# cnkuangshi/LightCTR

Hardware: AMD Instinct MI355X
Metric: examples/sec (whole node), FM training on synthetic Criteo-shaped sparse (higher is better)
Workload: dtype fp32; 1 GPU; model=FM k=16, ftrl fused update, global_batch=65536, num_features=16777216, num_fields=39, parallelism=single-gpu, hipGraph

## Files before the change

lightctr_amd/models/fm.py:

```python

from __future__ import annotations

from dataclasses import dataclass

import torch

from ..ops import fm_ref
from ..ops._extension import require_hip_ops, sort_ids, sort_ids_rec
from ..utils.checks import validate_csr_batch
from ..utils.metrics import auc_score


@dataclass
class FMHyper:
    num_features: int
    k: int = 16
    optimizer: str = "adagrad"
    lr: float = 0.1
    eps: float = 1e-8
    l2: float = 1e-5
    ftrl_alpha: float = 0.15
    ftrl_beta: float = 1.0
    ftrl_l1: float = 1e-4
    ftrl_l2: float = 1e-4
    ftrl_v: str = "adagrad"
    init_sigma: float = 0.01
    seed: int = 1234


class FMModel:

    def __init__(self, hyper: FMHyper, device: str = "cpu",
                 max_batch_nnz: int = 1 << 22):
        self.h = hyper
        self.device = torch.device(device)
        F, K = hyper.num_features, hyper.k
        assert K in (4, 8, 16, 32, 64), "K must divide the 64-lane wavefront"
        g = torch.Generator().manual_seed(hyper.seed)
        self.W = torch.zeros(F, device=self.device)
        self.V = (
            torch.randn(F, K, generator=g) * hyper.init_sigma
        ).to(self.device)
        self.gradW = torch.zeros_like(self.W)
        self.gradV = torch.zeros_like(self.V)
        self.nW = torch.zeros_like(self.W)
        self.nV = torch.zeros_like(self.V)
        if hyper.optimizer == "ftrl":
            self.zW = torch.zeros_like(self.W)
            self.zV = torch.zeros_like(self.V)
        nwords = (F + 63) // 64
        self.touched = torch.zeros(nwords, dtype=torch.int64, device=self.device)
        cap = min(F, max_batch_nnz)
        self.uniq = torch.zeros(cap, dtype=torch.int32, device=self.device)
        self.count = torch.zeros(1, dtype=torch.int32, device=self.device)
        self._use_hip = self.device.type == "cuda"
        self.backward_mode = "segment"
        self.segment_cap = 256
        self.fused_apply = False
        if self._use_hip:
            require_hip_ops()

    def forward(self, row_ptr, fids, vals):
        if self._use_hip:
            ops = require_hip_ops()
            pred, sumVX = ops.fm_forward(row_ptr, fids, vals, self.W, self.V)
        else:
            pred, sumVX = fm_ref.fm_forward_ref(row_ptr, fids, vals, self.W, self.V)
        return pred, sumVX

    def predict_proba(self, row_ptr, fids, vals):
        pred, _ = self.forward(row_ptr, fids, vals)
        return torch.sigmoid(torch.clamp(pred, -16, 16))

    def train_step(self, row_ptr, fids, vals, labels) -> torch.Tensor:
        B = row_ptr.numel() - 1
        scale = 1.0 / B
        validate_csr_batch(row_ptr, fids, vals, self.h.num_features)
        if self._use_hip:
            ops = require_hip_ops()
            if (self.backward_mode in ("segment", "segment_list")
                    and not self.fused_apply):
                tiled = (self.backward_mode == "segment"
                         and self._cap_tiles(ops))
                loss, dpred, sumVX, rec = ops.fm_forward_train(
                    row_ptr, fids, vals, self.W, self.V, labels, scale,
                    reset=self.count if tiled else None)
                self._segment_backward(ops, fids, sumVX, dpred, rec, tiled)
                return loss
            pred, sumVX = ops.fm_forward(row_ptr, fids, vals, self.W, self.V)
            loss, dpred = ops.logloss_grad(pred, labels, scale)
            if (self.backward_mode == "segment_emit"
                    and not self.fused_apply):
                self._segment_emit_backward(ops, row_ptr, fids, vals, sumVX,
                                            dpred)
                return loss
            if self.backward_mode in ("sorted", "segment", "segment_list",
                                      "segment_emit"):
                sorted_fids, perm = sort_ids(fids, self.h.num_features)
                gw, gv = ops.fm_backward_emit(row_ptr, fids, vals, self.V,
                                              sumVX, dpred)
                if self.fused_apply:
                    if (self.h.optimizer == "ftrl"
                            and self.h.ftrl_v == "adagrad"):
                        ops.fm_sorted_apply_fused(
                            sorted_fids, perm, gw, gv, self.gradW,
                            self.gradV, self.touched, self.W, self.V,
                            self.nW, self.nV, self.zW, None, 3,
                            self.h.ftrl_alpha, self.h.ftrl_beta,
                            self.h.ftrl_l1, self.h.ftrl_l2,
                            v_lr=self.h.lr, v_eps=self.h.eps,
                            v_l2=self.h.l2)
                    elif self.h.optimizer == "ftrl":
                        ops.fm_sorted_apply_fused(
                            sorted_fids, perm, gw, gv, self.gradW,
                            self.gradV, self.touched, self.W, self.V,
                            self.nW, self.nV, self.zW, self.zV, 2,
                            self.h.ftrl_alpha, self.h.ftrl_beta,
                            self.h.ftrl_l1, self.h.ftrl_l2)
                    else:
                        ops.fm_sorted_apply_fused(
                            sorted_fids, perm, gw, gv, self.gradW,
                            self.gradV, self.touched, self.W, self.V,
                            self.nW, self.nV, None, None, 1, self.h.lr,
                            self.h.eps, self.h.l2, 0.0)
                else:
                    ops.fm_sorted_apply(sorted_fids, perm, gw, gv,
                                        self.gradW, self.gradV,
                                        self.touched)
            else:
                ops.fm_backward(row_ptr, fids, vals, self.V, sumVX, dpred,
                                self.gradW, self.gradV, self.touched)
            self.count.zero_()
            ops.bitmap_compact(self.touched, self.uniq, self.count)
            live = self.uniq[: min(self.uniq.numel(), fids.numel())]
            self._sparse_apply(ops, live)
            return loss
        pred, sumVX = fm_ref.fm_forward_ref(row_ptr, fids, vals, self.W, self.V)
        loss, dpred = fm_ref.logloss_grad_ref(pred, labels, scale)
        gW, gV = fm_ref.fm_backward_ref(row_ptr, fids, vals, self.V, sumVX, dpred)
        self.gradW += gW
        self.gradV += gV
        uniq = torch.unique(fids.long()).int()
        if self.h.optimizer == "ftrl":
            fm_ref.ftrl_apply_ref(uniq, self.W, self.V, self.zW, self.nW,
                                  self.zV, self.nV, self.gradW, self.gradV,
                                  self.h.ftrl_alpha, self.h.ftrl_beta,
                                  self.h.ftrl_l1, self.h.ftrl_l2,
                                  v_adagrad=self.h.ftrl_v == "adagrad",
                                  v_lr=self.h.lr, v_eps=self.h.eps,
                                  v_l2=self.h.l2)
        else:
            fm_ref.adagrad_apply_ref(uniq, self.W, self.V, self.nW, self.nV,
                                     self.gradW, self.gradV, self.h.lr,
                                     self.h.eps, self.h.l2)
        return loss

    def _opt_mode(self) -> int:
        if self.h.optimizer != "ftrl":
            return 1
        return 3 if self.h.ftrl_v == "adagrad" else 2

    def _sparse_apply(self, ops, live):
        if self.h.optimizer == "ftrl":
            ops.fm_ftrl_apply(live, self.count, self.W, self.V,
                              self.zW, self.nW, self.zV, self.nV,
                              self.gradW, self.gradV, self.h.ftrl_alpha,
                              self.h.ftrl_beta, self.h.ftrl_l1,
                              self.h.ftrl_l2,
                              1 if self.h.ftrl_v == "adagrad" else 0,
                              self.h.lr, self.h.eps, self.h.l2)
        else:
            ops.fm_adagrad_apply(live, self.count, self.W, self.V,
                                 self.nW, self.nV, self.gradW, self.gradV,
                                 self.h.lr, self.h.eps, self.h.l2)

    def _cap_tiles(self, ops) -> bool:
        tile, cap = ops.fm_segment_tile(), int(self.segment_cap)
        return cap <= tile and tile % cap == 0

    def _segment_pieces(self, ops, sorted_fids, worklist=True):
        nnz = sorted_fids.numel()
        cap = int(self.segment_cap)
        if worklist:
            lists = tuple(ops.segment_worklist(sorted_fids, cap, self.count))
        else:
            lists = (cap,)
        spill = self.uniq[: min(self.uniq.numel(), nnz // cap + 1)]
        mode = self._opt_mode()
        if mode == 1:
            knobs = (self.h.lr, self.h.eps, self.h.l2, 0.0)
        else:
            knobs = (self.h.ftrl_alpha, self.h.ftrl_beta, self.h.ftrl_l1,
                     self.h.ftrl_l2)
        tail = (*lists, self.gradW, self.gradV, spill,
                self.count, self.W, self.V, self.nW, self.nV,
                self.zW if mode != 1 else None,
                self.zV if mode == 2 else None, mode, *knobs)
        kw = dict(v_lr=self.h.lr, v_eps=self.h.eps, v_l2=self.h.l2)
        return spill, tail, kw

    def _segment_backward(self, ops, fids, sumVX, dpred, rec, tiled):
        if fids.numel() == 0:
            return
        sorted_fids, sorted_rec = sort_ids_rec(fids, rec,
                                               self.h.num_features)
        spill, tail, kw = self._segment_pieces(ops, sorted_fids,
                                               worklist=not tiled)
        reduce = (ops.fm_segment_tile_rec if tiled
                  else ops.fm_segment_apply_rec)
        reduce(sorted_fids, sorted_rec, sumVX, dpred, *tail, **kw)
        self._sparse_apply(ops, spill)

    def _segment_emit_backward(self, ops, row_ptr, fids, vals, sumVX, dpred):
        if fids.numel() == 0:
            return
        sorted_fids, perm = sort_ids(fids, self.h.num_features)
        gw, gv = ops.fm_backward_emit(row_ptr, fids, vals, self.V, sumVX,
                                      dpred)
        spill, tail, kw = self._segment_pieces(ops, sorted_fids)
        ops.fm_segment_apply(sorted_fids, perm, tail[0], tail[1], gw, gv,
                             *tail[2:], **kw)
        self._sparse_apply(ops, spill)

    def state_dict(self) -> dict:
        d = {"W": self.W, "V": self.V, "nW": self.nW, "nV": self.nV,
             "hyper": self.h.__dict__}
        if self.h.optimizer == "ftrl":
            d["zW"], d["zV"] = self.zW, self.zV
        return d

    def save(self, path: str) -> None:
        torch.save(self.state_dict(), path)

    def load(self, path: str) -> None:
        d = torch.load(path, map_location=self.device, weights_only=True)
        self.W.copy_(d["W"])
        self.V.copy_(d["V"])
        self.nW.copy_(d["nW"])
        self.nV.copy_(d["nV"])
        if self.h.optimizer == "ftrl" and "zW" in d:
            self.zW.copy_(d["zW"])
            self.zV.copy_(d["zV"])


class FMTrainer:

    def __init__(self, dataset, hyper: FMHyper, device: str = "cpu",
                 batch_size: int = 256, epochs: int = 5):
        self.ds = dataset
        self.model = FMModel(hyper, device=device)
        self.batch_size = batch_size
        self.epochs = epochs
        self.device = torch.device(device)

    def train(self, log=print):
        ds = self.ds.to(self.device)
        N = ds.num_rows
        for ep in range(self.epochs):
            total_loss = 0.0
            nb = 0
            for s in range(0, N, self.batch_size):
                e = min(s + self.batch_size, N)
                b = ds.slice_rows(s, e)
                loss = self.model.train_step(b.row_ptr, b.fids, b.vals, b.labels)
                total_loss += float(loss.mean())
                nb += 1
            if log:
                log(f"epoch {ep}: loss={total_loss / max(nb, 1):.5f}")
        return self

    def evaluate(self, dataset=None) -> dict:
        ds = (dataset or self.ds).to(self.device)
        p = self.model.predict_proba(ds.row_ptr, ds.fids, ds.vals)
        loss = torch.nn.functional.binary_cross_entropy(
            p.clamp(1e-7, 1 - 1e-7), ds.labels
        )
        return {
            "auc": auc_score(p.cpu(), ds.labels.cpu()),
            "logloss": float(loss),
            "accuracy": float(((p > 0.5) == (ds.labels > 0.5)).float().mean()),
        }
```

lightctr_amd/ops/_extension.py:

```python

from __future__ import annotations

import torch

_hip_ops = None
_import_error: Exception | None = None

try:
    from . import _hip_ops as _ext

    _hip_ops = _ext
except ImportError as e:
    _import_error = e


def has_hip_ops() -> bool:
    return _hip_ops is not None


def require_hip_ops():
    if _hip_ops is None:
        raise ImportError(
            "lightctr_amd HIP extension (_hip_ops) is not built but a GPU "
            "op was requested. Build it in-tree with "
            "`PYTORCH_ROCM_ARCH=gfx950 python setup.py build_ext --inplace`. "
            f"Original import error: {_import_error!r}"
        )
    return _hip_ops


class _LazyOps:

    def __getattr__(self, name):
        return getattr(require_hip_ops(), name)


hip_ops = _LazyOps()


def sort_ids(fids, upper: int):
    end_bit = max(1, int(upper - 1).bit_length())
    return require_hip_ops().radix_sort_index(fids, end_bit)


def sort_ids_rec(fids, rec, upper: int):
    end_bit = max(1, int(upper - 1).bit_length())
    return require_hip_ops().radix_sort_rec(fids, rec, end_bit)
```

lightctr_amd/ops/csrc/bindings.cpp:

```cpp
#include <torch/extension.h>
#include <ATen/cuda/CUDAContext.h>
#include <c10/cuda/CUDAException.h>

#include <cstdint>
#include <cstdio>
#include <cstdlib>
#include <cstring>
#include <limits>
#include <stdexcept>
#include <string>
#include <vector>

#include "launchers.h"

namespace {

#define CHK(x, ...) TORCH_CHECK(x, __VA_ARGS__)

void check_cuda_f32(const at::Tensor& t, const char* name) {
  CHK(t.is_cuda(), name, " must be on GPU");
  CHK(t.scalar_type() == at::kFloat, name, " must be fp32");
  CHK(t.is_contiguous(), name, " must be contiguous");
}

// ... 1030 lines not shown
at::Tensor gemm_bf16(at::Tensor A, at::Tensor Bst,
                     c10::optional<at::Tensor> bias, int64_t M, int64_t N,
                     int64_t K, int64_t transA, int64_t transB, int64_t act,
                     bool emit_bf16) {
  const float* bias_ptr =
      check_gemm_args(A, Bst, bias, M, N, K, transA, transB, act);
  auto C = at::empty({M, N}, A.options().dtype(at::kFloat));
  at::Tensor Cbf;
  void* cbf_ptr = nullptr;
  if (emit_bf16) {
    Cbf = at::empty({M, N}, A.options());
    cbf_ptr = Cbf.data_ptr();
  }
  lightctr::gemm_bf16_launch(A.data_ptr(), Bst.data_ptr(), bias_ptr,
                             C.data_ptr<float>(), cbf_ptr, (int)M, (int)N,
                             (int)K, (int)transA, (int)transB, (int)act,
                             cur_stream());
  return C;
}

std::vector<at::Tensor> gemm_bf16_full(at::Tensor A, at::Tensor Bst,
                                       c10::optional<at::Tensor> bias,
                                       int64_t M, int64_t N, int64_t K,
                                       int64_t transA, int64_t transB,
                                       int64_t act) {
  const float* bias_ptr =
      check_gemm_args(A, Bst, bias, M, N, K, transA, transB, act);
  auto C = at::empty({M, N}, A.options().dtype(at::kFloat));
  auto Cbf = at::empty({M, N}, A.options());
  lightctr::gemm_bf16_launch(A.data_ptr(), Bst.data_ptr(), bias_ptr,
                             C.data_ptr<float>(), Cbf.data_ptr(), (int)M,
                             (int)N, (int)K, (int)transA, (int)transB,
                             (int)act, cur_stream());
  return {C, Cbf};
}

std::vector<at::Tensor> act_backward(at::Tensor dY, at::Tensor Y,
                                     int64_t act) {
  check_cuda_f32(dY, "dY");
  auto dZ = at::empty_like(dY);
  auto dZbf = at::empty_like(dY, dY.options().dtype(at::kBFloat16));
  lightctr::act_backward_launch(dY.data_ptr<float>(), Y.data_ptr<float>(),
                                dZ.data_ptr<float>(), dZbf.data_ptr(),
                                dY.numel(), (int)act, cur_stream());
  return {dZ, dZbf};
}

std::vector<at::Tensor> radix_sort_index(at::Tensor keys, int64_t end_bit) {
  check_cuda_i32(keys, "keys");
  CHK(end_bit >= 1 && end_bit <= 32, "end_bit in [1,32]");
  const int n = (int)keys.numel();
  auto sorted = at::empty_like(keys);
  auto perm = at::empty({n}, keys.options());
  auto iota = at::empty({n}, keys.options());
  lightctr::iota_i32_launch(iota.data_ptr<int>(), n, cur_stream());
  const unsigned long bytes =
      lightctr::radix_sort_pairs_i32_temp_bytes(n, (int)end_bit);
  auto temp = at::empty({(long)bytes}, keys.options().dtype(at::kByte));
  lightctr::radix_sort_pairs_i32_launch(
      temp.data_ptr(), bytes, keys.data_ptr<int>(), sorted.data_ptr<int>(),
      iota.data_ptr<int>(), perm.data_ptr<int>(), n, (int)end_bit,
      cur_stream());
  return {sorted, perm};
}

std::vector<at::Tensor> radix_sort_rec(at::Tensor keys, at::Tensor rec,
                                       int64_t end_bit) {
  check_cuda_i32(keys, "keys");
  CHK(end_bit >= 1 && end_bit <= 32, "end_bit in [1,32]");
  const int n = (int)keys.numel();
  check_cuda_rec(rec, n, "rec");
  auto sorted = at::empty_like(keys);
  auto sorted_rec = at::empty_like(rec);
  if (n == 0) return {sorted, sorted_rec};
  const unsigned long bytes =
      lightctr::radix_sort_pairs_rec_temp_bytes(n, (int)end_bit);
  auto temp = at::empty({(long)bytes}, keys.options().dtype(at::kByte));
  lightctr::radix_sort_pairs_rec_launch(
      temp.data_ptr(), bytes, keys.data_ptr<int>(), sorted.data_ptr<int>(),
      rec.data_ptr<int>(), sorted_rec.data_ptr<int>(), n, (int)end_bit,
      cur_stream());
  return {sorted, sorted_rec};
}

at::Tensor colsum(at::Tensor dZ) {
  check_cuda_f32(dZ, "dZ");
  const int M = (int)dZ.size(0), N = (int)dZ.size(1);
  auto db = at::empty({N}, dZ.options());
  lightctr::colsum_launch(dZ.data_ptr<float>(), db.data_ptr<float>(), M, N,
                          cur_stream());
  return db;
}

at::Tensor to_bf16(at::Tensor x) {
  check_cuda_f32(x, "x");
  auto y = at::empty_like(x, x.options().dtype(at::kBFloat16));
  lightctr::to_bf16_launch(x.data_ptr<float>(), y.data_ptr(), x.numel(),
                           cur_stream());
  return y;
}

void dense_adam(at::Tensor W, at::Tensor grad, at::Tensor m, at::Tensor v,
                c10::optional<at::Tensor> Wbf, c10::optional<at::Tensor> Wtbf,
                double lr, double beta1, double beta2, double eps,
                int64_t step, double l2) {
  check_cuda_f32(W, "W");
  const int rows = (int)W.size(0);
  const int cols = (int)(W.numel() / W.size(0));
  const float bc1 = 1.f - powf((float)beta1, (float)step);
  const float bc2 = 1.f - powf((float)beta2, (float)step);
  lightctr::dense_adam_launch(
      W.data_ptr<float>(), grad.data_ptr<float>(), m.data_ptr<float>(),
      v.data_ptr<float>(), Wbf.has_value() ? Wbf->data_ptr() : nullptr,
      Wtbf.has_value() ? Wtbf->data_ptr() : nullptr, rows, cols, (float)lr,
      (float)beta1, (float)beta2, (float)eps, bc1, bc2, (float)l2,
      cur_stream());
}

void dense_adagrad(at::Tensor W, at::Tensor grad, at::Tensor n,
                   c10::optional<at::Tensor> Wbf,
                   c10::optional<at::Tensor> Wtbf, double lr, double eps,
                   double l2) {
  check_cuda_f32(W, "W");
  const int rows = (int)W.size(0);
  const int cols = (int)(W.numel() / W.size(0));
  lightctr::dense_adagrad_launch(
      W.data_ptr<float>(), grad.data_ptr<float>(), n.data_ptr<float>(),
      Wbf.has_value() ? Wbf->data_ptr() : nullptr,
      Wtbf.has_value() ? Wtbf->data_ptr() : nullptr, rows, cols, (float)lr,
      (float)eps, (float)l2, cur_stream());
}


at::Tensor embed_gather(at::Tensor row_ptr, at::Tensor fids, at::Tensor vals,
                        at::Tensor E, int64_t nf) {
  check_cuda_i32(row_ptr, "row_ptr");
  check_cuda_i32(fids, "fids");
  check_cuda_f32(vals, "vals");
  check_cuda_f32(E, "E");
  CHK(E.dim() == 2, "E must be [F, K]");
  CHK(fids.numel() == vals.numel(), "fids/vals length mismatch");
  CHK(row_ptr.numel() >= 1, "row_ptr must hold B+1 offsets");
  CHK(nf >= 1, "nf must be >= 1");
  const int B = (int)row_ptr.numel() - 1;
  const int K = (int)E.size(1);
  check_embed_k(K);
  auto out = at::empty({B, nf * K}, E.options().dtype(at::kBFloat16));
  lightctr::embed_gather_launch(row_ptr.data_ptr<int>(), fids.data_ptr<int>(),
                                vals.data_ptr<float>(), E.data_ptr<float>(),
                                out.data_ptr(), (int)nf, B, K, cur_stream());
  return out;
}

std::vector<at::Tensor> embed_backward_emit(at::Tensor row_ptr,
                                            at::Tensor vals, at::Tensor dOut,
                                            at::Tensor dwide, int64_t nf,
                                            int64_t K) {
  check_cuda_i32(row_ptr, "row_ptr");
  check_cuda_f32(dOut, "dOut");
  check_cuda_f32(vals, "vals");
  check_cuda_f32(dwide, "dwide");
  check_embed_k(K);
  CHK(nf >= 1, "nf must be >= 1");
  const int B = (int)row_ptr.numel() - 1;
  CHK(dOut.numel() == (int64_t)B * nf * K, "dOut must be [B, nf*K]");
  const auto nnz = vals.numel();
// ... 494 lines not shown
  m.def("fm_segment_tile", &lightctr::fm_segment_tile,
        "entries per block of fm_segment_tile_rec");
  m.def("fm_segment_split", &lightctr::fm_segment_split,
        "longest unit one subgroup sums in fm_segment_tile_rec");
  m.def("ffm_forward", &ffm_forward, "FFM pairwise forward (LDS-staged)");
  m.def("ffm_forward_pp", &ffm_forward_pp, "lane-per-pair FFM forward");
  m.def("ffm_row_emit", &ffm_row_emit,
        "FFM per-row staged fp16 block emit -> (gw, gblocks)",
        py::arg("row_ptr"), py::arg("fields"), py::arg("fids"),
        py::arg("vals"), py::arg("V"), py::arg("dpred"),
        py::arg("scale") = 1.0);
  m.def("ffm_blocks_apply_f16", &ffm_blocks_apply_f16,
        "segment-reduce fp16 blocks into slabs (interior stores), "
        "optionally with the optimizer fused for interior runs",
        py::arg("sorted_fids"), py::arg("perm"), py::arg("gblocks"),
        py::arg("gw"), py::arg("gradW"), py::arg("gradV"),
        py::arg("touched"), py::arg("inv_scale") = 1.0,
        py::arg("opt_mode") = 0, py::arg("V") = py::none(),
        py::arg("W") = py::none(), py::arg("nW") = py::none(),
        py::arg("zW") = py::none(), py::arg("nV") = py::none(),
        py::arg("Vh") = py::none(), py::arg("p0") = 0.0,
        py::arg("p1") = 0.0, py::arg("p2") = 0.0, py::arg("p3") = 0.0,
        py::arg("q0") = 0.0, py::arg("q1") = 0.0, py::arg("q2") = 0.0);
  m.def("ffm_backward", &ffm_backward, "FFM fused pairwise backward scatter");
  m.def("ffm_sorted_backward", &ffm_sorted_backward,
        "FFM sorted segment-reduce backward (LDS block accumulate)");
  m.def("row_index", &row_index, "entry -> row index from row_ptr");
  m.def("ffm_block_lds_bytes", &lightctr::ffm_block_lds_bytes,
        "dynamic LDS per block of ffm_sorted_backward / ffm_block_emit",
        py::arg("nfields"), py::arg("K"));
  m.def("ffm_max_lds_per_block", &lightctr::ffm_max_lds_per_block,
        "per-block LDS limit of the current device, in bytes");
  m.def("ffm_block_emit", &ffm_block_emit,
        "FFM per-entry [nf,K] gradient blocks (wave/entry)");
  m.def("ffm_blocks_apply", &ffm_blocks_apply,
        "segment-reduce sorted FFM blocks into slabs");
  m.def("parse_libffm", &parse_libffm, "native libffm text parser",
        py::arg("path"), py::arg("max_rows") = -1);
  m.def("sparse_adagrad_apply", &sparse_adagrad_apply,
        "generic sparse fused Adagrad (runtime D)",
        py::arg("uniq"), py::arg("count"), py::arg("W"), py::arg("V"),
        py::arg("nW"), py::arg("nV"), py::arg("gradW"), py::arg("gradV"),
        py::arg("lr"), py::arg("eps"), py::arg("l2"),
        py::arg("Vh") = py::none());
  m.def("ps_apply", &ps_apply,
        "PS-side fused updater (sgd/adagrad/dcasgd/dcasgda)");
  m.def("ps_dense_check", &ps_dense_check,
        "PS dense push: non-finite scan of the payload -> flags[0]",
        py::arg("payload"), py::arg("scale"), py::arg("table"),
        py::arg("flags"));
  m.def("ps_dense_apply", &ps_dense_apply,
        "PS dense push: fused decode + updater over the slab, gated on "
        "flags[0]; a gated push bumps flags[1]. flags[0] is only what the "
        "last ps_dense_check left there: call ps_dense_check on the same "
        "payload, on the same stream, immediately before every call (as "
        "DenseTable.apply does) — called alone it acts on a stale flag",
        py::arg("payload"), py::arg("scale"), py::arg("table"),
        py::arg("slab"), py::arg("acc"), py::arg("shadow"),
        py::arg("flags"), py::arg("updater"), py::arg("lr"),
        py::arg("lam"), py::arg("eps"));
  m.def("ps_dense_pack", &ps_dense_pack,
        "PS dense pull: slab -> fp32/fp16 payload (+ shadow = slab)",
        py::arg("slab"), py::arg("shadow"), py::arg("fp16"));
  m.def("sparse_ftrl_apply", &sparse_ftrl_apply,
        "generic sparse fused FTRL (runtime D; optional Adagrad on V)",
        py::arg("uniq"), py::arg("count"), py::arg("W"), py::arg("V"),
        py::arg("zW"), py::arg("nW"), py::arg("zV"), py::arg("nV"),
        py::arg("gradW"), py::arg("gradV"), py::arg("alpha"),
        py::arg("beta"), py::arg("l1"), py::arg("l2"),
        py::arg("v_adagrad") = 0, py::arg("v_lr") = 0.05,
        py::arg("v_eps") = 1e-8, py::arg("v_l2") = 1e-5,
        py::arg("Vh") = py::none());
  m.def("gemm_bf16", &gemm_bf16, "MFMA bf16 GEMM (C fp32), fused bias+act");
  m.def("gemm_bf16_full", &gemm_bf16_full,
        "MFMA bf16 GEMM returning (C fp32, C bf16)");
  m.def("act_backward", &act_backward, "dZ = dY*act'(Y), + bf16 mirror");
  m.def("inv_perm_i32", &inv_perm_i32, "inverse permutation (int32)");
  m.def("radix_sort_index", &radix_sort_index,
        "bit-range radix sort -> (sorted, perm)");
  m.def("radix_sort_rec", &radix_sort_rec,
        "bit-range radix sort with [n,2] int32 records as payload -> "
        "(sorted, sorted_rec)",
        py::arg("keys"), py::arg("rec"), py::arg("end_bit"));
  m.def("colsum", &colsum, "bias gradient column sum");
  m.def("to_bf16", &to_bf16, "f32 -> bf16 convert");
  m.def("dense_adam", &dense_adam, "dense Adam + bf16 mirror refresh");
  m.def("dense_adagrad", &dense_adagrad,
        "dense Adagrad + bf16 mirror refresh");
  m.def("embed_gather", &embed_gather, "concat embedding gather -> bf16");
  m.def("embed_backward_emit", &embed_backward_emit,
        "per-entry embedding grads (gw, gv) for sorted apply");
  m.def("wide_forward", &wide_forward, "LR wide forward sum");
  m.def("w2v_negsample_step", &w2v_negsample_step,
        "fused CBOW negative-sampling train step (Hogwild)");
  m.def("quantile_encode", &quantile_encode, "int8 quantile encode");
  m.def("quantile_decode", &quantile_decode, "int8 quantile decode");
  m.def("lowbit_encode", &lowbit_encode, "1/2-bit sign quantize");
  m.def("lowbit_decode", &lowbit_decode, "1/2-bit dequantize");
  m.def("gbm_hist", &gbm_hist, "GBM per-node (grad,hess) histograms");
  m.def("gbm_forest", &gbm_forest,
        "compiled-forest inference: margin / leaf id / leaf feature id");
  m.def("gbm_forest_chunk_capacity", &lightctr::gbm_forest_chunk_capacity,
        "nodes per LDS chunk of the forest kernel");
  m.def("gbm_forest_max_register_classes",
        &lightctr::gbm_forest_max_register_classes,
        "largest class count with register accumulators");
  m.def("gbm_forest_rows_per_grid", &lightctr::gbm_forest_rows_per_grid,
        "rows one trip of the clamped grid covers");
  m.def("nfm_forward", &nfm_forward,
        "NFM bi-interaction fwd (wide, sumVX, vec, vec_bf16)");
  m.def("nfm_backward_emit", &nfm_backward_emit,
        "NFM per-entry grads for sorted apply");
  m.def("bitmap_compact", &bitmap_compact, "touched bitmap -> fid list");
  m.def("wg_probe", &wg_probe, "wgrad staging/tr-read debug probe");
  m.def("gemm_bf16_variant", &gemm_bf16_variant,
        "launch one named GEMM body directly; returns [C] or [C, Cbf]");
  m.def("gemm_bf16_route", &gemm_bf16_route,
        "name of the GEMM body the default dispatch picks");
  m.def("gemm_wgrad_bf16", &gemm_wgrad_bf16,
        "K-major x K-major wgrad GEMM (tr16 fragment reads)");
  m.def("im2col_bf16", &im2col_bf16,
        "fused unfold -> bf16 GEMM operand [B*L, C*k*k]");
  m.def("col2im", &col2im, "conv data-grad fold (gather form)");
  m.def("auc_hist_add", &auc_hist_add,
        "atomic pos/neg histogram accumulate for AUC");
  m.def("auc_scan", &auc_scan,
        "device scan of the AUC histogram -> {correct, P, N}");
  m.def("fm_adagrad_apply", &fm_adagrad_apply, "sparse fused Adagrad");
  m.def("fm_ftrl_apply", &fm_ftrl_apply,
        "sparse fused FTRL-proximal (optionally Adagrad on V)",
        py::arg("uniq"), py::arg("count"), py::arg("W"), py::arg("V"),
        py::arg("zW"), py::arg("nW"), py::arg("zV"), py::arg("nV"),
        py::arg("gradW"), py::arg("gradV"), py::arg("alpha"),
        py::arg("beta"), py::arg("l1"), py::arg("l2"),
        py::arg("v_adagrad") = 0, py::arg("v_lr") = 0.05,
        py::arg("v_eps") = 1e-8, py::arg("v_l2") = 1e-5);
  m.def("pq_lut", &pq_lut,
        "PQ distance tables [nq, n_sub, ncb]; metric 0 = l2, 1 = ip",
        py::arg("Q"), py::arg("centroids"), py::arg("metric"));
  m.def("pq_adc_topk", &pq_adc_topk,
        "ADC scan of uint8 codes + top-k -> (ids int32, dist fp32) [nq, k]",
        py::arg("lut"), py::arg("codes"), py::arg("ncb"), py::arg("k"));
  m.def("flat_topk", &flat_topk,
        "exact scan (or per-query candidate list) + top-k -> (ids, dist)",
        py::arg("X"), py::arg("Q"), py::arg("metric"), py::arg("k"),
        py::arg("cand") = py::none());
  m.def("knn_max_k", &lightctr::knn_max_k, "largest k of the top-k kernels");
  m.def("knn_max_sub", &lightctr::knn_max_sub,
        "largest n_sub of pq_adc_topk");
  m.def("knn_max_dim", &lightctr::knn_max_dim, "largest dim of flat_topk");
  m.def("knn_slice_rows", &lightctr::knn_slice_rows,
        "rows per block slice for n rows and nq queries", py::arg("n"),
        py::arg("nq"));
  m.def("forest_candidates", &forest_candidates,
        "best-first walk of a flattened random-projection forest -> "
        "candidate ids int32 [nq, width], -1 padded",
        py::arg("planes"), py::arg("bias"), py::arg("child"),
        py::arg("roots"), py::arg("leaf_off"), py::arg("leaf_items"),
        py::arg("Q"), py::arg("search_k"), py::arg("width"));
  m.def("forest_queue", &lightctr::forest_queue,
        "queue entries per query of forest_candidates");
  m.def("forest_max_search", &lightctr::forest_max_search,
        "largest search_k of forest_candidates");
}
```

lightctr_amd/ops/csrc/launchers.h:

```cpp
#pragma once

struct ihipStream_t;

namespace lightctr {

void fm_forward_launch(const int* row_ptr, const int* fids, const float* vals,
                       const float* W, const float* V, float* pred,
                       float* sumVX, int B, int K, ihipStream_t* stream);
void logloss_grad_launch(const float* pred, const float* label, float* loss,
                         float* dpred, float scale, int B,
                         ihipStream_t* stream);
void fm_backward_launch(const int* row_ptr, const int* fids, const float* vals,
                        const float* V, const float* sumVX, const float* dpred,
                        float* gradW, float* gradV, unsigned long long* touched,
                        int B, int K, ihipStream_t* stream);
void fm_backward_emit_launch(const int* row_ptr, const int* fids,
                             const float* vals, const float* V,
                             const float* sumVX, const float* dpred, float* gw,
                             float* gv, int B, int K, const int* pos,
                             ihipStream_t* stream);
void inv_perm_launch(const int* perm, int* inv, int n, ihipStream_t* stream);
void fm_sorted_apply_launch(const int* sorted_fids, const int* perm,
                            const float* gw, const float* gv, float* gradW,
                            float* gradV, unsigned long long* touched, int nnz,
// ... 203 lines not shown
                        int W, int k, int stride, int pad, int OH, int OW,
                        ihipStream_t* stream);
void col2im_launch(const float* dcol, float* dx, int B, int C, int H, int W,
                   int k, int stride, int pad, int OH, int OW,
                   ihipStream_t* stream);
void gemv_n1_launch(const void* A, const void* b, const float* bias,
                    float* C, void* Cbf, int M, int K, int act,
                    ihipStream_t* stream);
void wrowsum_m1_launch(const void* a, const void* Bst, float* C, int K,
                       int N, ihipStream_t* stream);
void outer_k1_launch(const void* A, const void* Bst, const float* bias,
                     float* C, void* Cbf, long M, long N, int act,
                     ihipStream_t* stream);
void act_backward_launch(const float* dY, const float* Y, float* dZ,
                         void* dZbf, long n, int act, ihipStream_t* stream);
void colsum_launch(const float* dZ, float* db, int M, int N,
                   ihipStream_t* stream);
void to_bf16_launch(const float* x, void* y, long n, ihipStream_t* stream);
void dense_adam_launch(float* W, const float* grad, float* m_t, float* v_t,
                       void* Wbf, void* Wtbf, int rows, int cols, float lr,
                       float beta1, float beta2, float eps, float bc1,
                       float bc2, float l2, ihipStream_t* stream);
void dense_adagrad_launch(float* W, const float* grad, float* n_t, void* Wbf,
                          void* Wtbf, int rows, int cols, float lr, float eps,
                          float l2, ihipStream_t* stream);

void embed_gather_launch(const int* row_ptr, const int* fids,
                         const float* vals, const float* E, void* out_bf,
                         int nf, int B, int K, ihipStream_t* stream);
void embed_backward_emit_launch(const int* row_ptr, const float* vals,
                                const float* dOut, const float* dwide,
                                float* gv, float* gw, int nf, int B, int K,
                                ihipStream_t* stream);
void wide_forward_launch(const int* row_ptr, const int* fids,
                         const float* vals, const float* W, float* wide,
                         int B, ihipStream_t* stream);
void nfm_forward_launch(const int* row_ptr, const int* fids, const float* vals,
                        const float* W, const float* V, float* wide,
                        float* sumVX, float* vec, void* vec_bf, int B, int K,
                        ihipStream_t* stream);
void w2v_negsample_launch(float* E, float* O, const long* centers,
                          const long* ctx, const long* negs, float* loss,
                          int B, int C, int N, int D, float lr, float scale,
                          ihipStream_t* stream);
void nfm_backward_emit_launch(const int* row_ptr, const int* fids,
                              const float* vals, const float* V,
                              const float* sumVX, const float* dvec,
                              const float* dwide, float* gw, float* gv, int B,
                              int K, ihipStream_t* stream);

void quantile_encode_launch(const float* x, unsigned char* code,
                            const float* table, int levels, long n,
                            ihipStream_t* stream);
void quantile_decode_launch(const unsigned char* code, float* x,
                            const float* table, int levels, long n,
                            ihipStream_t* stream);
void lowbit_encode_launch(const float* x, unsigned int* words, float thresh,
                          int bits, long n, ihipStream_t* stream);
void lowbit_decode_launch(const unsigned int* words, float* x, float lo,
                          float hi, int bits, long n, ihipStream_t* stream);

void ps_dense_check_launch(const void* payload, int wire, const float* scale,
                           const float* table, int levels, long n,
                           int* flags, ihipStream_t* stream);
void ps_dense_apply_launch(const void* payload, int wire, const float* scale,
                           const float* table, int levels, float* slab,
                           float* acc, float* shadow, long n, int updater,
                           float lr, float lam, float eps, int* flags,
                           ihipStream_t* stream);
void ps_dense_pack_launch(const float* slab, void* out, int fp16,
                          float* shadow, long n, ihipStream_t* stream);

void iota_i32_launch(int* out, int n, ihipStream_t* stream);
unsigned long radix_sort_pairs_i32_temp_bytes(int n, int end_bit);
void radix_sort_pairs_i32_launch(void* temp, unsigned long temp_bytes,
                                 const int* keys_in, int* keys_out,
                                 const int* vals_in, int* vals_out, int n,
                                 int end_bit, ihipStream_t* stream);
unsigned long radix_sort_pairs_rec_temp_bytes(int n, int end_bit);
void radix_sort_pairs_rec_launch(void* temp, unsigned long temp_bytes,
                                 const int* keys_in, int* keys_out,
                                 const int* rec_in, int* rec_out, int n,
                                 int end_bit, ihipStream_t* stream);
unsigned long segment_worklist_temp_bytes(int n);
void segment_worklist_launch(void* temp, unsigned long temp_bytes,
                             const int* sorted, int n, int cap,
                             int* piece_start, int* n_pieces, int* zero_me,
                             ihipStream_t* stream);

void gbm_hist_launch(const unsigned char* bins, const float* grad,
                     const float* hess, const int* node_of_row, float* hist,
                     int N, int D, int n_nodes, ihipStream_t* stream);
int gbm_forest_chunk_capacity();
int gbm_forest_max_register_classes();
long gbm_forest_rows_per_grid();
void gbm_forest_launch(const float* X, const void* nodes, const int* tree_off,
                       const int* tree_class, const int* leaf_base,
                       const void* chunks, int n_chunks, void* out, long N,
                       int D, int T, int K, int max_depth, int fid_offset,
                       int mode, ihipStream_t* stream);

int knn_max_k();
int knn_max_sub();
int knn_max_dim();
long knn_slice_rows(long n, long nq);
long pq_adc_lds_bytes(int n_sub, int ncb);
void pq_lut_launch(const float* Q, const float* C, float* lut, long nq,
                   int n_sub, int ncb, int d_sub, int ip,
                   ihipStream_t* stream);
void pq_adc_topk_launch(const float* lut, const unsigned char* codes,
                        long stride, long N, long nq, int n_sub, int ncb,
                        int k, long slice_rows, int n_slices, void* partial,
                        int* ids, float* dist, ihipStream_t* stream);
void flat_topk_launch(const float* X, long stride, long N, int dim,
                      const float* Q, long nq, const int* cand, long n_items,
                      int ip, int k, long slice_rows, int n_slices,
                      void* partial, int* ids, float* dist,
                      ihipStream_t* stream);
void knn_merge_launch(const void* partial, long nq, int n_slices, int k,
                      int dedup, int* ids, float* dist, ihipStream_t* stream);
int forest_queue();
int forest_max_search();
void forest_candidates_launch(const float* planes, const float* bias,
                              const int* child, const int* roots,
                              const int* leaf_off, const int* leaf_items,
                              const float* Q, int* cand, long nq, int dim,
                              int n_inner, int n_leaves, int T, long total,
                              int search_k, long width, ihipStream_t* stream);

}
```

lightctr_amd/ops/csrc/sort_kernels.hip:

```cpp
#include <rocprim/device/device_radix_sort.hpp>
#include <rocprim/device/device_select.hpp>
#include <rocprim/iterator/counting_iterator.hpp>
#include <rocprim/iterator/transform_iterator.hpp>

#include "common.h"

namespace lightctr {

__global__ void iota_i32_kernel(int* __restrict__ out, int n) {
  int i = blockIdx.x * blockDim.x + threadIdx.x;
  if (i < n) out[i] = i;
}

void iota_i32_launch(int* out, int n, hipStream_t stream) {
  if (n <= 0) return;
  int threads = 256;
  int blocks = (n + threads - 1) / threads;
  hipLaunchKernelGGL(iota_i32_kernel, dim3(blocks), dim3(threads), 0, stream,
                     out, n);
}

size_t radix_sort_pairs_i32_temp_bytes(int n, int end_bit) {
  size_t bytes = 0;
  (void)rocprim::radix_sort_pairs(nullptr, bytes, (const int*)nullptr,
                                  (int*)nullptr, (const int*)nullptr,
                                  (int*)nullptr, (size_t)n, 0u,
                                  (unsigned)end_bit, (hipStream_t)0, false);
  return bytes;
}

void radix_sort_pairs_i32_launch(void* temp, size_t temp_bytes,
                                 const int* keys_in, int* keys_out,
                                 const int* vals_in, int* vals_out, int n,
                                 int end_bit, hipStream_t stream) {
  LCTR_CHECK_HIP(rocprim::radix_sort_pairs(temp, temp_bytes, keys_in,
                                           keys_out, vals_in, vals_out,
                                           (size_t)n, 0u, (unsigned)end_bit,
                                           stream, false));
}

using SortRec = unsigned long long;

size_t radix_sort_pairs_rec_temp_bytes(int n, int end_bit) {
  size_t bytes = 0;
  (void)rocprim::radix_sort_pairs(nullptr, bytes, (const int*)nullptr,
                                  (int*)nullptr, (const SortRec*)nullptr,
                                  (SortRec*)nullptr, (size_t)n, 0u,
                                  (unsigned)end_bit, (hipStream_t)0, false);
  return bytes;
}

void radix_sort_pairs_rec_launch(void* temp, size_t temp_bytes,
                                 const int* keys_in, int* keys_out,
                                 const int* rec_in, int* rec_out, int n,
                                 int end_bit, hipStream_t stream) {
  LCTR_CHECK_HIP(rocprim::radix_sort_pairs(
      temp, temp_bytes, keys_in, keys_out, (const SortRec*)rec_in,
      (SortRec*)rec_out, (size_t)n, 0u, (unsigned)end_bit, stream, false));
}

struct PieceStartFlag {
  const int* sorted;
  int cap_mask;
  int* zero_me;
  __device__ bool operator()(int e) const {
    if (e == 0) {
      if (zero_me) *zero_me = 0;
      return true;
    }
    return (e & cap_mask) == 0 || sorted[e] != sorted[e - 1];
  }
};

using PieceFlagIter =
    rocprim::transform_iterator<rocprim::counting_iterator<int>,
                                PieceStartFlag, bool>;

size_t segment_worklist_temp_bytes(int n) {
  size_t bytes = 0;
  const rocprim::counting_iterator<int> idx(0);
  (void)rocprim::select(nullptr, bytes, idx,
                        PieceFlagIter(idx, PieceStartFlag{nullptr, 0, nullptr}),
                        (int*)nullptr, (int*)nullptr, (size_t)n,
                        (hipStream_t)0, false);
  return bytes;
}

void segment_worklist_launch(void* temp, size_t temp_bytes, const int* sorted,
                             int n, int cap, int* piece_start, int* n_pieces,
                             int* zero_me, hipStream_t stream) {
  const rocprim::counting_iterator<int> idx(0);
  LCTR_CHECK_HIP(rocprim::select(
      temp, temp_bytes, idx,
      PieceFlagIter(idx, PieceStartFlag{sorted, cap - 1, zero_me}),
      piece_start, n_pieces, (size_t)n, stream, false));
}

}
```

Measured before the change: 192.0 million examples/sec.

## Replace rocprim radix sort with custom onesweep sort for record-payload backward

```diff
diff --git a/lightctr_amd/models/fm.py b/lightctr_amd/models/fm.py
--- a/lightctr_amd/models/fm.py
+++ b/lightctr_amd/models/fm.py
@@ -57,6 +57,9 @@
         self.backward_mode = "segment"
         self.segment_cap = 256
         self.fused_apply = False
+        self.sort_impl = "onesweep"
+        self.sort_status = torch.zeros(1, dtype=torch.int32,
+                                       device=self.device)
         if self._use_hip:
             require_hip_ops()
 
@@ -202,8 +205,9 @@
     def _segment_backward(self, ops, fids, sumVX, dpred, rec, tiled):
         if fids.numel() == 0:
             return
-        sorted_fids, sorted_rec = sort_ids_rec(fids, rec,
-                                               self.h.num_features)
+        sorted_fids, sorted_rec = sort_ids_rec(
+            fids, rec, self.h.num_features, impl=self.sort_impl,
+            status=self.sort_status)
         spill, tail, kw = self._segment_pieces(ops, sorted_fids,
                                                worklist=not tiled)
         reduce = (ops.fm_segment_tile_rec if tiled
diff --git a/lightctr_amd/ops/_extension.py b/lightctr_amd/ops/_extension.py
--- a/lightctr_amd/ops/_extension.py
+++ b/lightctr_amd/ops/_extension.py
@@ -43,6 +43,11 @@
     return require_hip_ops().radix_sort_index(fids, end_bit)
 
 
-def sort_ids_rec(fids, rec, upper: int):
+def sort_ids_rec(fids, rec, upper: int, impl: str = "onesweep", status=None):
+    if impl not in ("onesweep", "rocprim"):
+        raise ValueError(f"unknown sort impl {impl!r}")
+    ops = require_hip_ops()
     end_bit = max(1, int(upper - 1).bit_length())
-    return require_hip_ops().radix_sort_rec(fids, rec, end_bit)
+    if impl == "onesweep" and end_bit <= 31 and fids.numel() < (1 << 30):
+        return ops.onesweep_sort_rec(fids, rec, end_bit, status)
+    return ops.radix_sort_rec(fids, rec, end_bit)
diff --git a/lightctr_amd/ops/csrc/bindings.cpp b/lightctr_amd/ops/csrc/bindings.cpp
--- a/lightctr_amd/ops/csrc/bindings.cpp
+++ b/lightctr_amd/ops/csrc/bindings.cpp
@@ -1136,6 +1136,40 @@
       cur_stream());
   return {sorted, sorted_rec};
 }
+
+std::vector<at::Tensor> onesweep_sort_rec(at::Tensor keys, at::Tensor rec,
+                                          int64_t end_bit,
+                                          c10::optional<at::Tensor> status) {
+  check_cuda_i32(keys, "keys");
+  CHK(end_bit >= 1 && end_bit <= 31, "end_bit in [1,31]");
+  CHK(keys.numel() < (1L << 30), "n must be below 2^30");
+  const int n = (int)keys.numel();
+  check_cuda_rec(rec, n, "rec");
+  if (status.has_value()) {
+    check_cuda_i32(*status, "status");
+    CHK(status->numel() >= 1, "status must hold one word");
+  }
+  auto sorted = at::empty_like(keys);
+  auto sorted_rec = at::empty_like(rec);
+  if (n == 0) return {sorted, sorted_rec};
+  auto st = status.has_value() ? *status : at::zeros({1}, keys.options());
+  const unsigned long bytes =
+      lightctr::onesweep_sort_work_bytes(n, (int)end_bit);
+  auto work = at::empty({(long)bytes}, keys.options().dtype(at::kByte));
+  at::Tensor keys_tmp, rec_tmp;
+  if (end_bit > 8) {
+    keys_tmp = at::empty_like(keys);
+    rec_tmp = at::empty_like(rec);
+  }
+  lightctr::onesweep_sort_rec_launch(
+      work.data_ptr(), keys.data_ptr<int>(), sorted.data_ptr<int>(),
+      end_bit > 8 ? keys_tmp.data_ptr<int>() : nullptr, rec.data_ptr<int>(),
+      sorted_rec.data_ptr<int>(),
+      end_bit > 8 ? rec_tmp.data_ptr<int>() : nullptr, n, (int)end_bit,
+      st.data_ptr<int>(), cur_stream());
+  return {sorted, sorted_rec};
+}
+
 
 at::Tensor colsum(at::Tensor dZ) {
   check_cuda_f32(dZ, "dZ");
@@ -1796,6 +1830,13 @@
         "bit-range radix sort with [n,2] int32 records as payload -> "
         "(sorted, sorted_rec)",
         py::arg("keys"), py::arg("rec"), py::arg("end_bit"));
+  m.def("onesweep_sort_rec", &onesweep_sort_rec,
+        "single-purpose onesweep sort with [n,2] int32 records as payload "
+        "-> (sorted, sorted_rec); same result as radix_sort_rec",
+        py::arg("keys"), py::arg("rec"), py::arg("end_bit"),
+        py::arg("status") = py::none());
+  m.def("onesweep_sort_tile", &lightctr::onesweep_sort_tile,
+        "entries per tile of onesweep_sort_rec");
   m.def("colsum", &colsum, "bias gradient column sum");
   m.def("to_bf16", &to_bf16, "f32 -> bf16 convert");
   m.def("dense_adam", &dense_adam, "dense Adam + bf16 mirror refresh");
diff --git a/lightctr_amd/ops/csrc/launchers.h b/lightctr_amd/ops/csrc/launchers.h
--- a/lightctr_amd/ops/csrc/launchers.h
+++ b/lightctr_amd/ops/csrc/launchers.h
@@ -309,6 +309,12 @@
                                  const int* keys_in, int* keys_out,
                                  const int* rec_in, int* rec_out, int n,
                                  int end_bit, ihipStream_t* stream);
+int onesweep_sort_tile();
+unsigned long onesweep_sort_work_bytes(int n, int end_bit);
+void onesweep_sort_rec_launch(void* work, const int* keys_in, int* keys_out,
+                              int* keys_tmp, const int* rec_in, int* rec_out,
+                              int* rec_tmp, int n, int end_bit, int* status,
+                              ihipStream_t* stream);
 unsigned long segment_worklist_temp_bytes(int n);
 void segment_worklist_launch(void* temp, unsigned long temp_bytes,
                              const int* sorted, int n, int cap,
diff --git a/lightctr_amd/ops/csrc/sort_kernels.hip b/lightctr_amd/ops/csrc/sort_kernels.hip
--- a/lightctr_amd/ops/csrc/sort_kernels.hip
+++ b/lightctr_amd/ops/csrc/sort_kernels.hip
@@ -1,3 +1,5 @@
+#include <algorithm>
+
 #include <rocprim/device/device_radix_sort.hpp>
 #include <rocprim/device/device_select.hpp>
 #include <rocprim/iterator/counting_iterator.hpp>
@@ -59,6 +61,309 @@
       (SortRec*)rec_out, (size_t)n, 0u, (unsigned)end_bit, stream, false));
 }
 
+constexpr int kOsRadix = 256;
+constexpr int kOsMaxPasses = 4;
+constexpr int kOsCtrlWords = kOsMaxPasses * kOsRadix + kOsMaxPasses;
+static_assert(kOsCtrlWords * 4 % 16 == 0, "memset block is 16-byte padded");
+constexpr unsigned kOsCountMask = 0x3fffffffu;
+constexpr unsigned kOsAggregate = 1u << 30;
+constexpr unsigned kOsPrefix = 2u << 30;
+constexpr unsigned kOsSpinLimit = 1u << 20;
+constexpr int kOsHistMaxThreads = 1024;
+constexpr int kOsHistMaxBlocks = 256;
+constexpr int kOsThreads = 512;
+constexpr int kOsItems = 8;
+constexpr int kOsWindow = 4;
+
+#define OS_RLX_AGENT __ATOMIC_RELAXED, __HIP_MEMORY_SCOPE_AGENT
+
+__global__ __launch_bounds__(kOsHistMaxThreads) void onesweep_hist_kernel(
+    const int* __restrict__ keys, int n, int passes, unsigned keymask,
+    unsigned* ghist, uint4* state, long state_vec4) {
+  __shared__ unsigned h[kOsMaxPasses * kOsRadix];
+  const int tid = threadIdx.x, threads = blockDim.x;
+  for (int i = tid; i < passes * kOsRadix; i += threads) h[i] = 0;
+  const long gstride = (long)gridDim.x * threads;
+  for (long i = (long)blockIdx.x * threads + tid; i < state_vec4; i += gstride)
+    state[i] = make_uint4(0u, 0u, 0u, 0u);
+  __syncthreads();
+  const int stride = (int)gstride;
+#pragma unroll 4
+  for (int i = blockIdx.x * threads + tid; i < n; i += stride) {
+    const unsigned k = (unsigned)keys[i] & keymask;
+#pragma unroll
+    for (int p = 0; p < kOsMaxPasses; ++p)
+      if (p < passes) atomicAdd(&h[p * kOsRadix + ((k >> (8 * p)) & 255u)], 1u);
+  }
+  __syncthreads();
+  for (int i = tid; i < passes * kOsRadix; i += threads) {
+    const unsigned c = h[i];
+    if (c) atomicAdd(&ghist[i], c);
+  }
+}
+
+__device__ __forceinline__ unsigned os_scan256(unsigned v, unsigned* wsum,
+                                               int tid) {
+  const int lane = tid & 63, w = tid >> 6;
+  unsigned incl = v;
+#pragma unroll
+  for (int o = 1; o < 64; o <<= 1) {
+    const unsigned t = __shfl_up(incl, o);
+    if (lane >= o) incl += t;
+  }
+  if (tid < kOsRadix && lane == 63) wsum[w] = incl;
+  __syncthreads();
+  unsigned add = 0;
+  if (tid < kOsRadix)
+    for (int k = 0; k < w; ++k) add += wsum[k];
+  return incl - v + add;
+}
+
+template <int THREADS, int IPT>
+constexpr int os_smem_bytes() {
+  constexpr int rank_bytes = (THREADS / 64) * kOsRadix * 12 + kOsRadix * 4;
+  constexpr int tile_bytes = THREADS * IPT * 12;
+  return (tile_bytes > rank_bytes ? tile_bytes : rank_bytes) + kOsRadix * 4 +
+         48;
+}
+
+template <int THREADS, int IPT>
+__global__ __launch_bounds__(THREADS) void onesweep_scatter_kernel(
+    const int* __restrict__ keys_in,
+    const unsigned long long* __restrict__ rec_in, int* __restrict__ keys_out,
+    unsigned long long* __restrict__ rec_out, int n, int shift,
+    unsigned keymask, const unsigned* __restrict__ ghist, unsigned* ticket,
+    unsigned* state, int* status) {
+  constexpr int TILE = THREADS * IPT, NW = THREADS / 64;
+  static_assert(THREADS >= kOsRadix && THREADS % 64 == 0, "one thread/digit");
+  constexpr int rank_bytes = NW * kOsRadix * 12 + kOsRadix * 4;
+  constexpr int main_bytes = TILE * 12 > rank_bytes ? TILE * 12 : rank_bytes;
+  extern __shared__ __attribute__((aligned(16))) unsigned char os_smem[];
+  unsigned long long* lrec = (unsigned long long*)os_smem;
+  unsigned* lkeys = (unsigned*)(os_smem + TILE * 8);
+  unsigned long long* wmask = (unsigned long long*)os_smem;
+  unsigned* wcnt = (unsigned*)(os_smem + NW * kOsRadix * 8);
+  unsigned* lbase = wcnt + NW * kOsRadix;
+  int* off = (int*)(os_smem + main_bytes);
+  unsigned* wsum_a = (unsigned*)(off + kOsRadix);
+  unsigned* wsum_b = wsum_a + 4;
+  unsigned* misc = wsum_b + 4;
+
+  const int tid = threadIdx.x, lane = tid & 63, w = tid >> 6;
+  if (tid == 0) {
+    misc[0] = atomicAdd(ticket, 1u);
+    misc[1] = 0;
+  }
+  for (int i = tid; i < NW * kOsRadix * 3; i += THREADS)
+    ((unsigned*)os_smem)[i] = 0;
+  __syncthreads();
+  const int tile = (int)misc[0];
+  const int tile_base = tile * TILE;
+  const int valid_n = min(TILE, n - tile_base);
+
+  unsigned key[IPT];
+  unsigned long long rec[IPT];
+  unsigned rank[IPT];
+  const int wbase = tile_base + w * (IPT * 64) + lane;
+#pragma unroll
+  for (int i = 0; i < IPT; ++i) {
+    const int idx = wbase + i * 64;
+    const bool v = idx < n;
+    key[i] = v ? (unsigned)keys_in[idx] : 0u;
+    rec[i] = v ? rec_in[idx] : 0ull;
+  }
+
+  unsigned* mycnt = wcnt + w * kOsRadix;
+  unsigned long long* mymask = wmask + w * kOsRadix;
+  const unsigned long long lane_bit = 1ull << lane;
+  const unsigned long long lanes_below = lane_bit - 1ull;
+#pragma unroll
+  for (int i = 0; i < IPT; ++i) {
+    const bool v = wbase + i * 64 < n;
+    const unsigned d = ((key[i] & keymask) >> shift) & 255u;
+    if (v) atomicOr(&mymask[d], lane_bit);
+    __builtin_amdgcn_fence(__ATOMIC_ACQ_REL, "wavefront");
+    __builtin_amdgcn_wave_barrier();
+    const unsigned long long m = v ? mymask[d] : 0ull;
+    const unsigned below = __popcll(m & lanes_below);
+    unsigned prev = 0;
+    if (v) prev = mycnt[d];
+    __builtin_amdgcn_fence(__ATOMIC_ACQ_REL, "wavefront");
+    __builtin_amdgcn_wave_barrier();
+    if (v && below == 0) {
+      mycnt[d] = prev + (unsigned)__popcll(m);
+      mymask[d] = 0ull;
+    }
+    __builtin_amdgcn_fence(__ATOMIC_ACQ_REL, "wavefront");
+    __builtin_amdgcn_wave_barrier();
+    rank[i] = prev + below;
+  }
+  __syncthreads();
+
+  unsigned cnt = 0;
+  if (tid < kOsRadix) {
+    for (int k = 0; k < NW; ++k) {
+      const unsigned c = wcnt[k * kOsRadix + tid];
+      wcnt[k * kOsRadix + tid] = cnt;
+      cnt += c;
+    }
+    if (tile != 0)
+      __hip_atomic_store(&state[(size_t)tile * kOsRadix + tid],
+                         kOsAggregate | cnt, OS_RLX_AGENT);
+  }
+  const unsigned lb = os_scan256(cnt, wsum_a, tid);
+  if (tid < kOsRadix) lbase[tid] = lb;
+  unsigned excl = 0;
+  if (tile == 0)
+    excl = os_scan256(tid < kOsRadix ? ghist[tid] : 0u, wsum_b, tid);
+  __syncthreads();
+
+#pragma unroll
+  for (int i = 0; i < IPT; ++i) {
+    const unsigned d = ((key[i] & keymask) >> shift) & 255u;
+    rank[i] += lbase[d] + wcnt[w * kOsRadix + d];
+  }
+  __syncthreads();
+#pragma unroll
+  for (int i = 0; i < IPT; ++i) {
+    if (wbase + i * 64 < n && rank[i] < (unsigned)TILE) {
+      lkeys[rank[i]] = key[i];
+      lrec[rank[i]] = rec[i];
+    }
+  }
+
+  if (tid < kOsRadix) {
+    bool fail = false;
+    if (tile != 0) {
+      int t = tile - 1;
+      unsigned spins = 0;
+      for (;;) {
+        unsigned s[kOsWindow];
+#pragma unroll
+        for (int k = 0; k < kOsWindow; ++k)
+          s[k] = t - k >= 0 ? __hip_atomic_load(
+                                  &state[(size_t)(t - k) * kOsRadix + tid],
+                                  OS_RLX_AGENT)
+                            : 0u;
+        int used = 0;
+        bool done = false;
+#pragma unroll
+        for (int k = 0; k < kOsWindow; ++k) {
+          const unsigned st = s[k] >> 30;
+          if (!done && used == k && st != 0u) {
+            excl += s[k] & kOsCountMask;
+            used = k + 1;
+            done = st == 2u;
+          }
+        }
+        if (done) break;
+        t -= used;
+        if (t < 0) {
+          fail = true;
+          break;
+        }
+        if (used == 0) {
+          ++spins;
+          if (spins >= kOsSpinLimit ||
+              ((spins & 1023u) == 0u &&
+               __hip_atomic_load(status, OS_RLX_AGENT) != 0)) {
+            fail = true;
+            break;
+          }
+          __builtin_amdgcn_s_sleep(1);
+        }
+      }
+    }
+    if (fail) {
+      atomicOr(status, 1);
+      misc[1] = 1u;
+    } else {
+      __hip_atomic_store(&state[(size_t)tile * kOsRadix + tid],
+                         kOsPrefix | ((excl + cnt) & kOsCountMask),
+                         OS_RLX_AGENT);
+    }
+    off[tid] = (int)(excl - lb);
+  }
+  __syncthreads();
+  if (misc[1]) return;
+
+  for (int j = tid; j < valid_n; j += THREADS) {
+    const unsigned k = lkeys[j];
+    const unsigned d = ((k & keymask) >> shift) & 255u;
+    const int dst = off[d] + j;
+    if ((unsigned)dst < (unsigned)n) {
+      keys_out[dst] = (int)k;
+      rec_out[dst] = lrec[j];
+    }
+  }
+}
+
+template <int THREADS, int IPT>
+void os_scatter_launch(int tiles, const int* keys_in, const SortRec* rec_in,
+                       int* keys_out, SortRec* rec_out, int n, int shift,
+                       unsigned keymask, const unsigned* ghist,
+                       unsigned* ticket, unsigned* state, int* status,
+                       hipStream_t stream) {
+  constexpr int smem = os_smem_bytes<THREADS, IPT>();
+  static_assert(smem <= 160 * 1024, "tile does not fit the LDS");
+  auto kernel = onesweep_scatter_kernel<THREADS, IPT>;
+  if (smem > 64 * 1024) {
+    static const hipError_t raised = hipFuncSetAttribute(
+        (const void*)kernel, hipFuncAttributeMaxDynamicSharedMemorySize, smem);
+    LCTR_CHECK_HIP(raised);
+  }
+  hipLaunchKernelGGL(kernel, dim3(tiles), dim3(THREADS), smem, stream, keys_in,
+                     rec_in, keys_out, rec_out, n, shift, keymask, ghist,
+                     ticket, state, status);
+}
+
+int onesweep_sort_tile() { return kOsThreads * kOsItems; }
+
+static int os_passes(int end_bit) { return (end_bit + 7) / 8; }
+
+size_t onesweep_sort_work_bytes(int n, int end_bit) {
+  const size_t tile = kOsThreads * kOsItems;
+  const size_t tiles = ((size_t)n + tile - 1) / tile;
+  return (size_t)kOsCtrlWords * 4 +
+         (size_t)os_passes(end_bit) * tiles * kOsRadix * 4;
+}
+
+void onesweep_sort_rec_launch(void* work, const int* keys_in, int* keys_out,
+                              int* keys_tmp, const int* rec_in, int* rec_out,
+                              int* rec_tmp, int n, int end_bit, int* status,
+                              hipStream_t stream) {
+  if (n <= 0) return;
+  const int passes = os_passes(end_bit);
+  const int tile = kOsThreads * kOsItems;
+  const int tiles = (n + tile - 1) / tile;
+  const unsigned keymask = (1u << end_bit) - 1u;
+  unsigned* ghist = (unsigned*)work;
+  unsigned* tickets = ghist + kOsMaxPasses * kOsRadix;
+  unsigned* state = ghist + kOsCtrlWords;
+  const size_t pass_words = (size_t)tiles * kOsRadix;
+  LCTR_CHECK_HIP(hipMemsetAsync(work, 0, (size_t)kOsCtrlWords * 4, stream));
+  const int hist_blocks = std::min(
+      kOsHistMaxBlocks,
+      (n + kOsHistMaxThreads * 8 - 1) / (kOsHistMaxThreads * 8));
+  hipLaunchKernelGGL(onesweep_hist_kernel, dim3(hist_blocks),
+                     dim3(kOsHistMaxThreads), 0, stream, keys_in, n, passes,
+                     keymask, ghist, (uint4*)state,
+                     (long)(passes * pass_words / 4));
+  const int* ksrc = keys_in;
+  const SortRec* rsrc = (const SortRec*)rec_in;
+  for (int p = 0; p < passes; ++p) {
+    const bool to_out = ((passes - 1 - p) & 1) == 0;
+    int* kdst = to_out ? keys_out : keys_tmp;
+    SortRec* rdst = (SortRec*)(to_out ? rec_out : rec_tmp);
+    os_scatter_launch<kOsThreads, kOsItems>(
+        tiles, ksrc, rsrc, kdst, rdst, n, 8 * p, keymask,
+        ghist + p * kOsRadix, tickets + p, state + p * pass_words, status,
+        stream);
+    ksrc = kdst;
+    rsrc = rdst;
+  }
+}
+
 struct PieceStartFlag {
   const int* sorted;
   int cap_mask;
```

Measured after the change: 204.6 million examples/sec, median of 6. +6.6%, better.
